# ku-fpg/ecc-ldpc

Hardware: AMD Instinct MI355X
Metric: decoded info Mbit/s @ 50 BP iters, jpl.4096.4.5, Eb/N0=2 dB (higher is better)
Workload: dtype f32; 1 GPU; jpl.4096.4.5 rate 4/5 (4096,5120) minsum flooding BP, 50 iters, Eb/N0=2.0 dB, 65536 frames/GPU/step; code_name=ldpc/hip-minsum/jpl.4096.4.5/50/4/5, batch_per_gpu=65536, parallelism=frames sharded over 1 GPU(s), tallies all-reduced

## Files before the change

ecc_ldpc_amd/csrc/fused_rows.h:

```cpp
#pragma once
#include "fused_common.h"
#ifndef LDPC_DEVICE_ONLY
#include "generated_tables.h"
#endif

namespace ldpc {

template <typename CT, int SZ>
struct DynRow {
    ctab_t p;
    __device__ __forceinline__ uint32_t lo(int k) const { return p[k] & 0xffffu; }
    __device__ __forceinline__ uint32_t hi(int k) const { return p[k] >> 16; }
};
template <typename CT, int SZ, class T, int EBEG>
struct StatRow {
    static constexpr uint32_t CPW = QcGeom<SZ>::CPW, V = QcGeom<SZ>::V, ES = sizeof(CT);
    __device__ __forceinline__ constexpr uint32_t lo(int k) const { return T::rot[EBEG + k] * CPW * ES; }
    __device__ __forceinline__ constexpr uint32_t hi(int k) const { return T::bc[EBEG + k] * V * ES; }
};
struct DynTab {
    ctab_t p;
    template <typename CT, int SZ, int EBEG> __device__ __forceinline__ DynRow<CT, SZ> row() const { return DynRow<CT, SZ>{p + EBEG}; }
    __device__ __forceinline__ DynTab rebase(uint32_t z) const { return DynTab{p + z}; }
};
template <class T>
struct StatTab {
    using Table = T;
    template <typename CT, int SZ, int EBEG> __device__ __forceinline__ StatRow<CT, SZ, T, EBEG> row() const { return {}; }
    __device__ __forceinline__ StatTab rebase(uint32_t) const { return {}; }
};
template <class Tab> struct IsStatic : std::false_type {};
template <class T> struct IsStatic<StatTab<T>> : std::true_type {};

template <class T>
struct Rounds {
    static constexpr int round_of(int e) {
        int c = 0;
        for (int j = e + 1; j < T::NEDGE; j++) c += (T::bc[j] == T::bc[e]) ? 1 : 0;
        return c;
    }
    static constexpr int num_rounds() {
        int m = 0;
        for (int e = 0; e < T::NEDGE; e++) m = round_of(e) + 1 > m ? round_of(e) + 1 : m;
        return m;
    }
    static constexpr int count(int q) {
        int c = 0;
        for (int e = 0; e < T::NEDGE; e++) c += round_of(e) == q ? 1 : 0;
        return c;
    }
    static constexpr int round0_edge(int bc) {
        for (int e = T::NEDGE - 1; e >= 0; e--)
            if (T::bc[e] == bc) return e;
        return -1;
    }
    static constexpr int nth(int q, int i) {
        int c = 0;
        for (int e = T::NEDGE - 1; e >= 0; e--)
            if (round_of(e) == q) { if (c == i) return e; c++; }
        return -1;
    }
};

template <typename CT, int SZ, class T, int Q, int I0, int I1>
__device__ __forceinline__ void round_chunk_b(char *lds, uint32_t p4, uint32_t vmask, const CT *msg, const CT *orig_rot) {
    constexpr uint32_t CPW = SZ >= 64 ? 1 : 64 / SZ, V = SZ * CPW, ES = sizeof(CT);
    asm volatile("" : "+v"(p4));
    if constexpr (Q == 0) {
        static_for<I0, I1>([&](auto ic) {
            constexpr int i = decltype(ic)::value;
            constexpr int e = Rounds<T>::nth(Q, i);
            lds_st<CT>(lds + T::bc[e] * V * ES, (p4 + T::rot[e] * CPW * ES) & vmask, msg[e] + orig_rot[T::bc[e]]);
        });
        return;
    }
    CT cur[I1 - I0];
    uint32_t adr[I1 - I0];
    static_for<I0, I1>([&](auto ic) {
        constexpr int i = decltype(ic)::value;
        constexpr int e = Rounds<T>::nth(Q, i);
        adr[i - I0] = (p4 + T::rot[e] * CPW * ES) & vmask;
        cur[i - I0] = lds_ld<CT>(lds + T::bc[e] * V * ES, adr[i - I0]);
    });
    static_for<I0, I1>([&](auto ic) {
        constexpr int i = decltype(ic)::value;
        constexpr int e = Rounds<T>::nth(Q, i);
        lds_st<CT>(lds + T::bc[e] * V * ES, adr[i - I0], msg[e] + cur[i - I0]);
    });
}
template <typename CT, int SZ, class T, int Q, int I0>
__device__ __forceinline__ void round_b(char *lds, uint32_t p4, uint32_t vmask, const CT *msg, const CT *orig_rot) {
    constexpr int CNT = Rounds<T>::count(Q), CH = 8;
    if constexpr (I0 < CNT) {
        round_chunk_b<CT, SZ, T, Q, I0, (I0 + CH < CNT ? I0 + CH : CNT)>(lds, p4, vmask, msg, orig_rot);
        round_b<CT, SZ, T, Q, I0 + CH>(lds, p4, vmask, msg, orig_rot);
    }
}

template <int RPL, int HSTEP>
__device__ __forceinline__ uint32_t row_addr(uint32_t a0, uint32_t p4, uint32_t lo, uint32_t vmask, int h) {
    if (h == 0) return a0;
    if (RPL == 2) return a0 ^ (uint32_t)HSTEP;
    return qc_wrap((p4 + HSTEP * h) + lo, vmask);
}

template <typename CT, int VARIANT, int D, int RPL, int HSTEP, bool SYNDROME_ONLY, class Row>
__device__ __forceinline__ bool rows_a(const char *lds, Row tabrow, uint32_t p4, uint32_t vmask, CT *msg) {
    asm volatile("" : "+v"(p4));
    if constexpr (SYNDROME_ONLY) LDPC_COLD_PATH();
    CT l[RPL][D];
    static_for<0, D>([&](auto kc) {
        constexpr int k = decltype(kc)::value;
        const uint32_t lo = tabrow.lo(k), hi = tabrow.hi(k);
        uint32_t a0 = qc_wrap(p4 + lo, vmask);
#pragma unroll
        for (int h = 0; h < RPL; h++) l[h][k] = lds_ld<CT>(lds + hi, row_addr<RPL, HSTEP>(a0, p4, lo, vmask, h));
    });
    bool any = false;
#pragma unroll
    for (int h = 0; h < RPL; h++) {
        bool par = false;
#pragma unroll
        for (int k = 0; k < D; k++) par ^= (l[h][k] > CT(0));
        any |= par;
    }
    if constexpr (SYNDROME_ONLY) return any;
#pragma unroll
    for (int h = 0; h < RPL; h++) {
        CT *m = msg + h * D;
        if constexpr (VARIANT == LDPC_V_MINSUM && sizeof(CT) == 4) {
            static_assert(D >= 2, "min-sum needs degree >= 2");
            uint32_t X = 0;
            float m1 = INFINITY, m2 = INFINITY;
            static_for<0, D>([&](auto kc) {
                constexpr int k = decltype(kc)::value;
                float t = l[h][k] - m[k];
                m[k] = t;
                X ^= __float_as_uint(t);
                float a = fabsf(t);
                m2 = __builtin_amdgcn_fmed3f(m1, m2, a);
                m1 = fminf(m1, a);
            });
            const uint32_t flip = (X ^ ((D & 1) ? 0x80000000u : 0u)) & 0x80000000u;
            const uint32_t c1 = __float_as_uint(0.75f * m1) ^ flip;
            const uint32_t c2 = __float_as_uint(0.75f * m2) ^ flip;
            static_for<0, D>([&](auto kc) {
                constexpr int k = decltype(kc)::value;
                float t = m[k];
                uint32_t c = (fabsf(t) == m1) ? c2 : c1;
                uint32_t tb = __float_as_uint(t);
                m[k] = __uint_as_float(__builtin_amdgcn_bitop3_b32(c, tb, 0x80000000u, 0x78));
            });
        } else {
            CT t[D];
#pragma unroll
            for (int k = 0; k < D; k++) t[k] = l[h][k] - m[k];
            cn_update<CT, VARIANT, D>(t);
#pragma unroll
            for (int k = 0; k < D; k++) m[k] = t[k];
        }
    }
    return any;
}

template <typename CT, int D, int RPL, int HSTEP, class Row>
__device__ __forceinline__ void rows_b(char *lds, Row tabrow, uint32_t p4, uint32_t vmask, const CT *msg) {
    asm volatile("" : "+v"(p4));
    CT cur[RPL][D];
    uint32_t adr[D];
    static_for<0, D>([&](auto kc) {
        constexpr int k = decltype(kc)::value;
        const uint32_t lo = tabrow.lo(k), hi = tabrow.hi(k);
        adr[k] = qc_wrap(p4 + lo, vmask);
#pragma unroll
        for (int h = 0; h < RPL; h++) cur[h][k] = lds_ld<CT>(lds + hi, row_addr<RPL, HSTEP>(adr[k], p4, lo, vmask, h));
    });
    static_for<0, D>([&](auto kc) {
        constexpr int k = decltype(kc)::value;
        const uint32_t lo = tabrow.lo(k), hi = tabrow.hi(k);
#pragma unroll
        for (int h = 0; h < RPL; h++) lds_st<CT>(lds + hi, row_addr<RPL, HSTEP>(adr[k], p4, lo, vmask, h), msg[h * D + k] + cur[h][k]);
    });
}

}
```

ecc_ldpc_amd/csrc/fused_split.hip:

```cpp
#include <stdio.h>

#ifndef SPLIT_ORIG_LDS
#define SPLIT_ORIG_LDS 12
#endif
#include "fused_split_body.h"

#ifndef SPLIT_WAVES_PER_EU
#define SPLIT_WAVES_PER_EU 4
#endif
#ifndef SPLIT_TANH_WAVES_PER_EU
#define SPLIT_TANH_WAVES_PER_EU 3
#endif

namespace ldpc {

template <typename CT, int VARIANT, class Plan, int SZ, class T>
__global__ __launch_bounds__((SplitGeom<Plan, SZ>::THREADS), (VARIANT == LDPC_V_TANH ? SPLIT_TANH_WAVES_PER_EU : SPLIT_WAVES_PER_EU))
void fused_split_kernel(FusedArgs A) {
    split_kernel_body<CT, VARIANT, Plan, SZ, T>(A);
}

bool fused_split_has(int variant, int dtype, int sz, int static_id) {
    if (dtype != LDPC_F32 || !(variant == LDPC_MINSUM || variant == LDPC_TANH)) return false;
    return (sz == 128 && static_id == 2) || (sz == 32 && static_id == 1);
}

template <int VARIANT, int SZ, class T>
static void launch_split(hipStream_t st, FusedArgs &a) {
    using G = SplitGeom<PlanAR4JA45, SZ>;
    const int grid = (a.batch + G::CPW - 1) / G::CPW;
    hipLaunchKernelGGL((fused_split_kernel<float, VARIANT, PlanAR4JA45, SZ, T>), dim3(grid), dim3(G::THREADS), 0, st, a);
}

int fused_split_launch(int variant, int sz, hipStream_t st, FusedArgs &a, KernelTimer *timer, LaunchInfo *info) {
    if (info && !a.step_mode) {
        snprintf(info->name, sizeof(info->name), "ldpc::fused_split_kernel<float, %d, ldpc::PlanAR4JA45, %d, ", variant == LDPC_MINSUM ? LDPC_V_MINSUM : LDPC_V_TANH, sz);
        info->threads = sz == 128 ? SplitGeom<PlanAR4JA45, 128>::THREADS : SplitGeom<PlanAR4JA45, 32>::THREADS;
        info->frames_per_wg = sz == 128 ? SplitGeom<PlanAR4JA45, 128>::CPW : SplitGeom<PlanAR4JA45, 32>::CPW;
    }
    if (timer && !a.step_mode) timer->begin(st);
#ifdef SPLIT_ABLATION_MINSUM128
    launch_split<LDPC_V_MINSUM, 128, TabJpl4096>(st, a);
#else
    if (sz == 128) {
        if (variant == LDPC_MINSUM) launch_split<LDPC_V_MINSUM, 128, TabJpl4096>(st, a);
        else launch_split<LDPC_V_TANH, 128, TabJpl4096>(st, a);
    } else {
        if (variant == LDPC_MINSUM) launch_split<LDPC_V_MINSUM, 32, TabJpl1024>(st, a);
        else launch_split<LDPC_V_TANH, 32, TabJpl1024>(st, a);
    }
#endif
    if (timer && !a.step_mode) timer->end(st);
    hipError_t e = hipGetLastError();
    if (e != hipSuccess) return set_error(LDPC_EHIP, "fused_split launch: %s", hipGetErrorString(e));
    return LDPC_OK;
}

}
```

ecc_ldpc_amd/csrc/fused_split_body.h:

```cpp
#pragma once
#include "fused_rows.h"

#ifndef SPLIT_ORIG_REGS
#define SPLIT_ORIG_REGS 1
#endif
#ifndef SPLIT_ORIG_LDS
#define SPLIT_ORIG_LDS 0
#endif
#ifndef SPLIT_PRIO_A
#define SPLIT_PRIO_A 2
#endif
#ifndef SPLIT_PRIO_B
#define SPLIT_PRIO_B 0
#endif
#ifndef SPLIT_CH
#define SPLIT_CH 12
#endif
#ifndef SPLIT_CH_SMALL
#define SPLIT_CH_SMALL 24
#endif

namespace ldpc {

#ifndef SPLIT_RESULT_PACKED
#define SPLIT_RESULT_PACKED 1
#endif
template <int NB, bool PACKED = (SPLIT_RESULT_PACKED && NB <= 22)> struct SplitResult;
template <int NB> struct SplitResult<NB, true> {
    struct Bits {
        uint32_t w = 0;
        __device__ __forceinline__ void set(int i, bool b) { w |= (b ? 1u : 0u) << i; }
        __device__ __forceinline__ uint32_t get(int i) const { return (w >> i) & 1u; }
    } bits;
    __device__ __forceinline__ void converge_at(int n) { bits.w = (1u << 22) | ((uint32_t)n << 23); }
    __device__ __forceinline__ bool converged() const { return (bits.w >> 22) & 1u; }
    __device__ __forceinline__ int turn() const { return (int)(bits.w >> 23); }
};
template <int NB> struct SplitResult<NB, false> {
    struct Bits {
        uint32_t w[(NB + 31) / 32] = {};
        __device__ __forceinline__ void set(int i, bool b) { w[i >> 5] |= (b ? 1u : 0u) << (i & 31); }
        __device__ __forceinline__ uint32_t get(int i) const { return (w[i >> 5] >> (i & 31)) & 1u; }
    } bits;
    uint32_t flag = 0;
    __device__ __forceinline__ void converge_at(int n) { bits = Bits{}; flag = 0x80000000u | (uint32_t)n; }
    __device__ __forceinline__ bool converged() const { return flag >> 31; }
    __device__ __forceinline__ int turn() const { return (int)(flag & 0x7fffffffu); }
};

template <class Plan, class T>
struct Split {
    static constexpr int br_of(int e) {
        int br = 0;
        for (int b = 0; b < Plan::NBR; b++) if (Plan::ebeg(b) <= e) br = b;
        return br;
    }
    static constexpr int owner_br(int br) { return Plan::owner_br(br); }
    static constexpr int owner(int e) { return owner_br(br_of(e)); }
    static constexpr int slot(int e) {
        int c = 0;
        for (int j = 0; j < e; j++) c += owner(j) == owner(e) ? 1 : 0;
        return c;
    }
    static constexpr int nmsg(int p) {
        int c = 0;
        for (int e = 0; e < T::NEDGE; e++) c += owner(e) == p ? 1 : 0;
        return c;
    }
    static constexpr int max_over_groups(int (*f)(int)) { int m = 0; for (int g = 0; g < Plan::NP; g++) m = f(g) > m ? f(g) : m; return m; }
    static constexpr int NMSG = max_over_groups(nmsg);
    static constexpr int oowner(int bc) { return owner(Rounds<T>::round0_edge(bc)); }
    static constexpr int oslot(int bc) {
        int c = 0;
        for (int j = 0; j < bc; j++) c += oowner(j) == oowner(bc) ? 1 : 0;
        return c;
    }
    static constexpr int norig(int p) {
        int c = 0;
        for (int bc = 0; bc < T::NBC; bc++) c += oowner(bc) == p ? 1 : 0;
        return c;
    }
    static constexpr int NORIG = max_over_groups(norig);
    static constexpr int count(int q, int p) {
        int c = 0;
        for (int e = 0; e < T::NEDGE; e++) c += (Rounds<T>::round_of(e) == q && owner(e) == p) ? 1 : 0;
        return c;
    }
    static constexpr int nth(int q, int p, int i) {
        int c = 0;
        for (int e = T::NEDGE - 1; e >= 0; e--)
            if (Rounds<T>::round_of(e) == q && owner(e) == p) { if (c == i) return e; c++; }
        return -1;
    }
};

template <typename CT, int VARIANT, class Plan, int SZ, class T>
struct SplitLds {
    static constexpr int V = QcGeom<SZ>::V, VT = QcGeom<SZ>::VT, THREADS = Plan::NP * VT, NW = THREADS / 64, ES = sizeof(CT);
    static constexpr int LAM_BYTES = (Plan::NBC * V * ES + 15) / 16 * 16;
    static constexpr int ORIG_OFF = LAM_BYTES + (4 * NW + 15) / 16 * 16;
    static constexpr int NOL_WANT = (VARIANT == LDPC_V_MINSUM && ES == 4 && SZ >= 64 && SPLIT_ORIG_REGS) ? SPLIT_ORIG_LDS : 0;
    static constexpr int NOL = NOL_WANT < Split<Plan, T>::NORIG ? NOL_WANT : Split<Plan, T>::NORIG;
    static constexpr int BYTES = NOL ? ORIG_OFF + NOL * THREADS * ES : LAM_BYTES + 4 * NW;
    static constexpr uint32_t orig_at(int P, int os) { return ORIG_OFF + (uint32_t)(os * THREADS + P * VT) * ES; }
};

template <typename CT, int VARIANT, int SZ, class Plan, class T, int P, int Q, int I0, int I1>
__device__ __forceinline__ void split_round_chunk(char *lds, uint32_t p4, uint32_t vmask, const CT *msg, const CT *orig_rot, const float *gllr, uint32_t r0) {
    using S = Split<Plan, T>;
    using L = SplitLds<CT, VARIANT, Plan, SZ, T>;
    constexpr uint32_t ES = sizeof(CT), CPW = QcGeom<SZ>::CPW, V = QcGeom<SZ>::V;
    asm volatile("" : "+v"(p4));
    if constexpr (Q == 0) {
        static_for<I0, I1>([&](auto ic) {
            constexpr int e = S::nth(Q, P, decltype(ic)::value);
            constexpr int ms = S::slot(e), os = S::oslot(T::bc[e]);
            CT o;
            if constexpr (SPLIT_ORIG_REGS && os < L::NOL) o = lds_ld<CT>(lds + L::orig_at(P, os), p4);
            else if constexpr (SPLIT_ORIG_REGS) o = orig_rot[os]; else o = (CT)gllr[T::bc[e] * SZ + ((r0 + T::rot[e]) % SZ)];
            lds_st<CT>(lds + T::bc[e] * V * ES, qc_wrap(p4 + T::rot[e] * CPW * ES, vmask), msg[ms] + o);
        });
        return;
    }
    CT cur[I1 - I0];
    uint32_t adr[I1 - I0];
    static_for<I0, I1>([&](auto ic) {
        constexpr int i = decltype(ic)::value;
        constexpr int e = S::nth(Q, P, i);
        adr[i - I0] = qc_wrap(p4 + T::rot[e] * CPW * ES, vmask);
        cur[i - I0] = lds_ld<CT>(lds + T::bc[e] * V * ES, adr[i - I0]);
    });
    static_for<I0, I1>([&](auto ic) {
        constexpr int i = decltype(ic)::value;
        constexpr int e = S::nth(Q, P, i);
        constexpr int ms = S::slot(e);
        lds_st<CT>(lds + T::bc[e] * V * ES, adr[i - I0], msg[ms] + cur[i - I0]);
    });
    asm volatile("" ::: "memory");
}
template <typename CT, int VARIANT, int SZ, class Plan, class T, int P, int Q, int I0>
__device__ __forceinline__ void split_round(char *lds, uint32_t p4, uint32_t vmask, const CT *msg, const CT *orig_rot, const float *gllr, uint32_t r0) {
    constexpr int CNT = Split<Plan, T>::count(Q, P), CH = SZ < 64 ? SPLIT_CH_SMALL : SPLIT_CH;
    if constexpr (I0 < CNT) {
        split_round_chunk<CT, VARIANT, SZ, Plan, T, P, Q, I0, (I0 + CH < CNT ? I0 + CH : CNT)>(lds, p4, vmask, msg, orig_rot, gllr, r0);
        split_round<CT, VARIANT, SZ, Plan, T, P, Q, I0 + CH>(lds, p4, vmask, msg, orig_rot, gllr, r0);
    }
}

template <typename CT, int VARIANT, class Plan, int SZ, class T, int P>
__device__ __forceinline__ void split_body(const FusedArgs &A, char *lds, const uint32_t tid) {
    using S = Split<Plan, T>;
    constexpr int CPW = QcGeom<SZ>::CPW, V = QcGeom<SZ>::V, VT = QcGeom<SZ>::VT;
    constexpr int N = Plan::NBC * SZ, THREADS = Plan::NP * VT, NW = THREADS / 64;
    constexpr uint32_t ES = sizeof(CT), vmask = V * ES - 1;
    constexpr int LAM_BYTES = (Plan::NBC * V * (int)ES + 15) / 16 * 16;
    if constexpr (VT != V) { if ((tid % VT) >= (uint32_t)V) return; }
    const uint32_t p4 = (tid % VT) * ES;
    struct Where {
        uint32_t sub, r0; long long frame; bool valid; size_t fN, fE;
        __device__ __forceinline__ Where(uint32_t p, int batch) {
            asm volatile("" : "+v"(p));
            const uint32_t lane = p / ES;
            sub = lane % CPW;
            r0 = lane / CPW;
            frame = (long long)blockIdx.x * CPW + sub;
            valid = frame < batch;
            fN = (size_t)(valid ? frame : 0) * N;
            fE = (size_t)(valid ? frame : 0) * Plan::NEDGE * SZ;
        }
    };
    const Where w0(p4, A.batch);
    const uint32_t r0 = w0.r0;
    const size_t fN = w0.fN, fE = w0.fE;
    CT msg[S::NMSG];
    CT orig[SPLIT_ORIG_REGS ? S::NORIG : 1];
#pragma unroll
    for (int i = 0; i < S::NMSG; i++) msg[i] = CT(0);
#pragma unroll
    for (int i = 0; i < (SPLIT_ORIG_REGS ? S::NORIG : 1); i++) orig[i] = CT(0);
    using L = SplitLds<CT, VARIANT, Plan, SZ, T>;
    static_assert(L::NOL == 0 || L::BYTES <= 65536, "LDS of one workgroup");
    auto put_orig = [&](int os, CT v) {
        if (os < L::NOL) lds_st<CT>(lds + L::orig_at(P, os), p4, v); else orig[os] = v;
    };
    typename SplitResult<(Plan::NBC + Plan::NP - 1) / Plan::NP>::Bits obits{};
    with_llr_format(A.llr_fmt, [&](auto fc) {
        constexpr int FMT = decltype(fc)::value;
        static_for<0, Plan::NBC>([&](auto bcc) {
            constexpr int bc = decltype(bcc)::value;
            if constexpr ((bc % Plan::NP) == P) {
                CT v = maybe_round_f16<CT>(load_llr_as<CT, FMT>(A.llr, fN + bc * SZ + r0), A.llr_round16);
                obits.set(bc / Plan::NP, v > CT(0));
                if (A.step_mode) v = (CT)A.st_lam[fN + bc * SZ + r0];
                lds_st<CT>(lds, p4 + (bc * V * ES), v);
            }
        });
        if (A.step_mode) {
            static_for<0, Plan::NBC>([&](auto bcc) {
                constexpr int bc = decltype(bcc)::value;
                if constexpr (SPLIT_ORIG_REGS && S::oowner(bc) == P) {
                    constexpr int e0 = Rounds<T>::round0_edge(bc);
                    constexpr int os = S::oslot(bc);
                    put_orig(os, maybe_round_f16<CT>(load_llr_as<CT, FMT>(A.llr, fN + bc * SZ + ((r0 + T::rot[e0]) % SZ)), A.llr_round16));
                }
            });
        }
    });
    if (A.step_mode) {
        static_for<0, Plan::NBR>([&](auto brc) {
            constexpr int br = decltype(brc)::value;
            if constexpr (S::owner_br(br) == P) {
                constexpr int D = Plan::deg(br);
                static_for<0, D>([&](auto kc) {
                    constexpr int k = decltype(kc)::value;
                    constexpr int ms = S::slot(Plan::ebeg(br) + k);
                    msg[ms] = (CT)A.st_ne_in[fE + (size_t)SZ * Plan::ebeg(br) + (size_t)D * r0 + k];
                });
            }
        });
    }
    __syncthreads();
    if (!A.step_mode) {
        static_for<0, Plan::NBC>([&](auto bcc) {
            constexpr int bc = decltype(bcc)::value;
            if constexpr (SPLIT_ORIG_REGS && S::oowner(bc) == P) {
                constexpr int e0 = Rounds<T>::round0_edge(bc);
                constexpr int os = S::oslot(bc);
                put_orig(os, lds_ld<CT>(lds + bc * V * ES, qc_wrap(p4 + T::rot[e0] * CPW * ES, vmask)));
            }
        });
    }

    volatile uint32_t *flags = reinterpret_cast<volatile uint32_t *>(lds + LAM_BYTES);
    constexpr uint32_t FULL = (1u << CPW) - 1;
    uint32_t done = 0;
#pragma unroll
    for (int s2 = 0; s2 < CPW; s2++) done |= ((long long)blockIdx.x * CPW + s2 < A.batch) ? 0u : (1u << s2);
    SplitResult<(Plan::NBC + Plan::NP - 1) / Plan::NP> res;
    res.bits = obits;
    const int turns = A.step_mode ? 1 : A.max_iters;

    for (int n = 0;; n++) {
        if (done == FULL) break;
        if (A.trace && !((done >> ((p4 / ES) % CPW)) & 1u)) {
            LDPC_COLD_PATH();
            const Where w(p4, A.batch);
            static_for<0, Plan::NBC>([&](auto bcc) {
                constexpr int bc = decltype(bcc)::value;
                if constexpr ((bc % Plan::NP) == P)
                    A.trace[((size_t)w.frame * (A.max_iters + 1) + n) * N + bc * SZ + w.r0] = (double)lds_ld<CT>(lds, p4 + (bc * V * ES));
            });
        }
        const bool last = (n >= turns);
        bool unsat = false;
        static_for<0, Plan::NBR>([&](auto brc) {
            constexpr int br = decltype(brc)::value;
            if constexpr (S::owner_br(br) == P) {
                constexpr int D = Plan::deg(br), ms0 = S::slot(Plan::ebeg(br));
                StatRow<CT, SZ, T, Plan::ebeg(br)> row;
                if (last) unsat |= rows_a<CT, VARIANT, D, 1, 0, true>(lds, row, p4, vmask, (CT *)nullptr);
                else unsat |= rows_a<CT, VARIANT, D, 1, 0, false>(lds, row, p4, vmask, &msg[ms0]);
            }
        });
        const unsigned long long ub = __ballot(unsat);
        uint32_t wbits = 0;
#pragma unroll
        for (int s2 = 0; s2 < CPW; s2++) {
            unsigned long long m = 0;
            for (int i = 0; i < 64; i += CPW) m |= 1ull << i;
            wbits |= ((ub & (m << s2)) != 0ull) ? (1u << s2) : 0u;
        }
        if ((tid & 63) == 0) flags[tid >> 6] = wbits;
        __syncthreads();
        uint32_t fbits = 0;
#pragma unroll
        for (int w = 0; w < NW; w++) fbits |= flags[w];
        fbits = __builtin_amdgcn_readfirstlane(fbits);
        if (A.step_mode) {
            const Where w(p4, A.batch);
            if (w.valid && w.r0 == 0 && P == 0) A.st_syn[w.frame] = ((fbits >> w.sub) & 1u) ? 0 : 1;
        } else {
            uint32_t newly = ~fbits & ~done & FULL;
            if constexpr (kVetoesNonFinite<CT, VARIANT>) {
                if (newly != 0u) {
                    LDPC_COLD_PATH();
                    bool nf = false;
                    if ((newly >> ((p4 / ES) % CPW)) & 1u)
                        static_for<0, Plan::NBC>([&](auto bcc) {
                            constexpr int bc = decltype(bcc)::value;
                            if constexpr ((bc % Plan::NP) == P) nf |= not_finite(lds_ld<CT>(lds, p4 + (bc * V * ES)));
                        });
                    __syncthreads();
                    const unsigned long long vb = __ballot(nf);
                    uint32_t vbits = 0;
#pragma unroll
                    for (int s2 = 0; s2 < CPW; s2++) {
                        unsigned long long m = 0;
                        for (int i = 0; i < 64; i += CPW) m |= 1ull << i;
                        vbits |= ((vb & (m << s2)) != 0ull) ? (1u << s2) : 0u;
                    }
                    if ((tid & 63) == 0) flags[tid >> 6] = vbits;
                    __syncthreads();
                    uint32_t veto = 0;
#pragma unroll
                    for (int w = 0; w < NW; w++) veto |= flags[w];
                    veto = __builtin_amdgcn_readfirstlane(veto) & newly;
                    __syncthreads();
                    done |= veto;
                    newly &= ~veto;
                }
            }
            if ((newly >> ((p4 / ES) % CPW)) & 1u) {
                LDPC_COLD_PATH();
                res.converge_at(n);
                static_for<0, Plan::NBC>([&](auto bcc) {
                    constexpr int bc = decltype(bcc)::value;
                    if constexpr ((bc % Plan::NP) == P) {
                        CT v = lds_ld<CT>(lds, p4 + (bc * V * ES));
                        res.bits.set(bc / Plan::NP, v > CT(0));
                    }
                });
                if (A.final_lam) {
                    const Where w(p4, A.batch);
                    static_for<0, Plan::NBC>([&](auto bcc) {
                        constexpr int bc = decltype(bcc)::value;
                        if constexpr ((bc % Plan::NP) == P) A.final_lam[w.fN + bc * SZ + w.r0] = (double)lds_ld<CT>(lds, p4 + (bc * V * ES));
                    });
                }
            }
            done |= newly;
            if (CPW > 1 && newly != 0u && done != FULL) __syncthreads();
        }
        if (last) break;
        if (done != FULL) {
            __builtin_amdgcn_s_setprio(SPLIT_PRIO_B);
            static_for<0, Rounds<T>::num_rounds()>([&](auto qc) {
                split_round<CT, VARIANT, SZ, Plan, T, P, decltype(qc)::value, 0>(lds, p4, vmask, msg, orig, reinterpret_cast<const float *>(A.llr) + fN, r0);
                __syncthreads();
            });
            __builtin_amdgcn_s_setprio(SPLIT_PRIO_A);
        }
        if (A.step_mode) break;
    }

    const Where w(p4, A.batch);
    if (!w.valid) return;
    if (A.step_mode) {
        static_for<0, Plan::NBC>([&](auto bcc) {
            constexpr int bc = decltype(bcc)::value;
            if constexpr ((bc % Plan::NP) == P) A.final_lam[w.fN + bc * SZ + w.r0] = (double)lds_ld<CT>(lds, p4 + (bc * V * ES));
        });
        static_for<0, Plan::NBR>([&](auto brc) {
            constexpr int br = decltype(brc)::value;
            if constexpr (S::owner_br(br) == P) {
                constexpr int D = Plan::deg(br);
                static_for<0, D>([&](auto kc) {
                    constexpr int k = decltype(kc)::value;
                    constexpr int ms = S::slot(Plan::ebeg(br) + k);
                    A.st_ne_out[w.fE + (size_t)SZ * Plan::ebeg(br) + (size_t)D * w.r0 + k] = (double)msg[ms];
                });
            }
        });
        return;
    }
    const bool converged = res.converged();
    if (converged) {
        static_for<0, Plan::NBC>([&](auto bcc) {
            constexpr int bc = decltype(bcc)::value;
            if constexpr ((bc % Plan::NP) == P) A.bits[w.fN + bc * SZ + w.r0] = res.bits.get(bc / Plan::NP);
        });
    } else {
        static_for<0, Plan::NBC>([&](auto bcc) {
            constexpr int bc = decltype(bcc)::value;
            if constexpr ((bc % Plan::NP) == P) A.bits[w.fN + bc * SZ + w.r0] = res.bits.get(bc / Plan::NP);
        });
        if (A.final_lam) {
            with_llr_format(A.llr_fmt, [&](auto fc) {
                constexpr int FMT = decltype(fc)::value;
                static_for<0, Plan::NBC>([&](auto bcc) {
                    constexpr int bc = decltype(bcc)::value;
                    if constexpr ((bc % Plan::NP) == P) {
                        const size_t gi = w.fN + bc * SZ + w.r0;
                        A.final_lam[gi] = (double)maybe_round_f16<CT>(load_llr_as<CT, FMT>(A.llr, gi), A.llr_round16);
                    }
                });
            });
        }
    }
    if (w.r0 == 0 && P == 0) {
        if (A.iters) A.iters[w.frame] = converged ? res.turn() : turns;
        if (A.conv) A.conv[w.frame] = converged ? 1 : 0;
    }
}

template <class Plan, int SZ> struct SplitGeom {
    static constexpr int CPW = QcGeom<SZ>::CPW, V = QcGeom<SZ>::V, VT = QcGeom<SZ>::VT, THREADS = Plan::NP * VT, NW = THREADS / 64;
    static_assert(THREADS <= 1024, "a frame's wave groups must fit one workgroup");
};

template <typename CT, int VARIANT, class Plan, int SZ, class T>
__device__ __forceinline__ void split_kernel_body(const FusedArgs &A) {
    using G = SplitGeom<Plan, SZ>;
    static_assert(SZ >= 2, "circulant size");
    __shared__ __attribute__((aligned(16))) char lds[SplitLds<CT, VARIANT, Plan, SZ, T>::BYTES];
    const uint32_t tid = threadIdx.x;
    const uint32_t pair = __builtin_amdgcn_readfirstlane(tid / G::VT);
    static_for<0, Plan::NP>([&](auto pc) {
        constexpr int P = decltype(pc)::value;
        if (pair == (uint32_t)P) split_body<CT, VARIANT, Plan, SZ, T, P>(A, lds, tid);
    });
}

}
```

Baseline: 14760 Mbit/s.

## Specialise split kernel per wave with compile-time circulant addresses and negated lambda

Instantiates the split decoder body once per 64-lane wave, so circulant rotation offsets become compile-time constants and the modulo wrap is dropped wherever a wave's rotated window cannot wrap. It also stores lambda negated, so the syndrome parity becomes an XOR of sign bits and the variable-node update folds the sign, moves the syndrome flags to an explicit LDS address space, and raises the number of orig slots kept in LDS. The aim is fewer VALU address and compare instructions per iteration, at the cost of many more template instantiations, larger code and more instruction-cache pressure.

```diff
diff --git a/ecc_ldpc_amd/csrc/fused_rows.h b/ecc_ldpc_amd/csrc/fused_rows.h
--- a/ecc_ldpc_amd/csrc/fused_rows.h
+++ b/ecc_ldpc_amd/csrc/fused_rows.h
@@ -11,12 +11,33 @@
     ctab_t p;
     __device__ __forceinline__ uint32_t lo(int k) const { return p[k] & 0xffffu; }
     __device__ __forceinline__ uint32_t hi(int k) const { return p[k] >> 16; }
+    static constexpr bool nowrap(int) { return false; }
+    static constexpr bool any_wrap(int) { return true; }
 };
 template <typename CT, int SZ, class T, int EBEG>
 struct StatRow {
     static constexpr uint32_t CPW = QcGeom<SZ>::CPW, V = QcGeom<SZ>::V, ES = sizeof(CT);
     __device__ __forceinline__ constexpr uint32_t lo(int k) const { return T::rot[EBEG + k] * CPW * ES; }
     __device__ __forceinline__ constexpr uint32_t hi(int k) const { return T::bc[EBEG + k] * V * ES; }
+    static constexpr bool nowrap(int) { return false; }
+    static constexpr bool any_wrap(int) { return true; }
+};
+template <int SZ, int WV>
+struct WaveRot {
+    static_assert(WV < 0 || (QcGeom<SZ>::CPW == 1 && SZ % 64 == 0), "wave-specialised addresses: whole waves of one frame");
+    static constexpr uint32_t rot(uint32_t r) { return WV < 0 ? r * QcGeom<SZ>::CPW : (64u * WV + r) % SZ; }
+    static constexpr bool nowrap(uint32_t r) { return WV >= 0 && rot(r) + 63 < SZ; }
+};
+template <typename CT, int SZ, class T, int EBEG, int WV>
+struct StatRowW {
+    static constexpr uint32_t V = QcGeom<SZ>::V, ES = sizeof(CT);
+    __device__ __forceinline__ constexpr uint32_t lo(int k) const { return WaveRot<SZ, WV>::rot(T::rot[EBEG + k]) * ES; }
+    __device__ __forceinline__ constexpr uint32_t hi(int k) const { return T::bc[EBEG + k] * V * ES; }
+    static constexpr bool nowrap(int k) { return WaveRot<SZ, WV>::nowrap(T::rot[EBEG + k]); }
+    static constexpr bool any_wrap(int d) {
+        for (int k = 0; k < d; k++) if (!nowrap(k)) return true;
+        return false;
+    }
 };
 struct DynTab {
     ctab_t p;
@@ -104,25 +125,40 @@
     return qc_wrap((p4 + HSTEP * h) + lo, vmask);
 }
 
-template <typename CT, int VARIANT, int D, int RPL, int HSTEP, bool SYNDROME_ONLY, class Row>
+template <typename CT, int VARIANT, int D, int RPL, int HSTEP, bool SYNDROME_ONLY, bool NEG = false, class Row>
 __device__ __forceinline__ bool rows_a(const char *lds, Row tabrow, uint32_t p4, uint32_t vmask, CT *msg) {
-    asm volatile("" : "+v"(p4));
+    const uint32_t b4 = p4;
+    if constexpr (Row::any_wrap(D)) asm volatile("" : "+v"(p4));
     if constexpr (SYNDROME_ONLY) LDPC_COLD_PATH();
     CT l[RPL][D];
     static_for<0, D>([&](auto kc) {
         constexpr int k = decltype(kc)::value;
         const uint32_t lo = tabrow.lo(k), hi = tabrow.hi(k);
-        uint32_t a0 = qc_wrap(p4 + lo, vmask);
+        uint32_t a0;
+        if constexpr (Row::nowrap(k)) a0 = b4 + lo; else a0 = qc_wrap(p4 + lo, vmask);
 #pragma unroll
         for (int h = 0; h < RPL; h++) l[h][k] = lds_ld<CT>(lds + hi, row_addr<RPL, HSTEP>(a0, p4, lo, vmask, h));
     });
     bool any = false;
-#pragma unroll
-    for (int h = 0; h < RPL; h++) {
-        bool par = false;
-#pragma unroll
-        for (int k = 0; k < D; k++) par ^= (l[h][k] > CT(0));
-        any |= par;
+    if constexpr (NEG) {
+        static_assert(VARIANT == LDPC_V_MINSUM && sizeof(CT) == 4, "negated lam: the f32 min-sum form only");
+        uint32_t odd = 0;
+#pragma unroll
+        for (int h = 0; h < RPL; h++) {
+            uint32_t px = 0;
+#pragma unroll
+            for (int k = 0; k < D; k++) px ^= __float_as_uint(l[h][k]);
+            odd |= px;
+        }
+        any = (odd >> 31) != 0u;
+    } else {
+#pragma unroll
+        for (int h = 0; h < RPL; h++) {
+            bool par = false;
+#pragma unroll
+            for (int k = 0; k < D; k++) par ^= (l[h][k] > CT(0));
+            any |= par;
+        }
     }
     if constexpr (SYNDROME_ONLY) return any;
 #pragma unroll
@@ -134,7 +170,7 @@
             float m1 = INFINITY, m2 = INFINITY;
             static_for<0, D>([&](auto kc) {
                 constexpr int k = decltype(kc)::value;
-                float t = l[h][k] - m[k];
+                float t = NEG ? (-l[h][k]) - m[k] : l[h][k] - m[k];
                 m[k] = t;
                 X ^= __float_as_uint(t);
                 float a = fabsf(t);
diff --git a/ecc_ldpc_amd/csrc/fused_split.hip b/ecc_ldpc_amd/csrc/fused_split.hip
--- a/ecc_ldpc_amd/csrc/fused_split.hip
+++ b/ecc_ldpc_amd/csrc/fused_split.hip
@@ -1,7 +1,19 @@
 #include <stdio.h>
 
 #ifndef SPLIT_ORIG_LDS
-#define SPLIT_ORIG_LDS 12
+#define SPLIT_ORIG_LDS 13
+#endif
+#ifndef SPLIT_WAVE_SPEC
+#define SPLIT_WAVE_SPEC 1
+#endif
+#ifndef SPLIT_WAVE_PHASES
+#define SPLIT_WAVE_PHASES 1
+#endif
+#ifndef SPLIT_FLAGS_LDS
+#define SPLIT_FLAGS_LDS 1
+#endif
+#ifndef SPLIT_NEG_LAM
+#define SPLIT_NEG_LAM 1
 #endif
 #include "fused_split_body.h"
 
diff --git a/ecc_ldpc_amd/csrc/fused_split_body.h b/ecc_ldpc_amd/csrc/fused_split_body.h
--- a/ecc_ldpc_amd/csrc/fused_split_body.h
+++ b/ecc_ldpc_amd/csrc/fused_split_body.h
@@ -7,6 +7,18 @@
 #ifndef SPLIT_ORIG_LDS
 #define SPLIT_ORIG_LDS 0
 #endif
+#ifndef SPLIT_WAVE_SPEC
+#define SPLIT_WAVE_SPEC 0
+#endif
+#ifndef SPLIT_WAVE_PHASES
+#define SPLIT_WAVE_PHASES 3
+#endif
+#ifndef SPLIT_FLAGS_LDS
+#define SPLIT_FLAGS_LDS 0
+#endif
+#ifndef SPLIT_NEG_LAM
+#define SPLIT_NEG_LAM 0
+#endif
 #ifndef SPLIT_PRIO_A
 #define SPLIT_PRIO_A 2
 #endif
@@ -21,6 +33,21 @@
 #endif
 
 namespace ldpc {
+
+template <typename CT, int VARIANT, int SZ>
+constexpr bool kSplitWholeWaves = VARIANT == LDPC_V_MINSUM && sizeof(CT) == 4 && QcGeom<SZ>::CPW == 1 && QcGeom<SZ>::VT == QcGeom<SZ>::V && QcGeom<SZ>::VT > 64;
+template <bool LDS_AS> struct SynFlags;
+template <> struct SynFlags<false> {
+    volatile uint32_t *p;
+    __device__ __forceinline__ explicit SynFlags(char *at) : p(reinterpret_cast<volatile uint32_t *>(at)) {}
+    __device__ __forceinline__ volatile uint32_t &operator[](uint32_t w) const { return p[w]; }
+};
+template <> struct SynFlags<true> {
+    typedef __attribute__((address_space(3))) volatile uint32_t *ptr_t;
+    ptr_t p;
+    __device__ __forceinline__ explicit SynFlags(char *at) : p((ptr_t)at) {}
+    __device__ __forceinline__ __attribute__((address_space(3))) volatile uint32_t &operator[](uint32_t w) const { return p[w]; }
+};
 
 #ifndef SPLIT_RESULT_PACKED
 #define SPLIT_RESULT_PACKED 1
@@ -105,20 +132,32 @@
     static constexpr uint32_t orig_at(int P, int os) { return ORIG_OFF + (uint32_t)(os * THREADS + P * VT) * ES; }
 };
 
-template <typename CT, int VARIANT, int SZ, class Plan, class T, int P, int Q, int I0, int I1>
-__device__ __forceinline__ void split_round_chunk(char *lds, uint32_t p4, uint32_t vmask, const CT *msg, const CT *orig_rot, const float *gllr, uint32_t r0) {
+template <typename CT, int VARIANT, int SZ, class Plan, class T, int P, int WV, int Q, int I0, int I1>
+__device__ __forceinline__ void split_round_chunk(char *lds, const uint32_t b4, uint32_t vmask, const CT *msg, const CT *orig_rot, const float *gllr, uint32_t r0) {
     using S = Split<Plan, T>;
     using L = SplitLds<CT, VARIANT, Plan, SZ, T>;
-    constexpr uint32_t ES = sizeof(CT), CPW = QcGeom<SZ>::CPW, V = QcGeom<SZ>::V;
-    asm volatile("" : "+v"(p4));
+    using R = WaveRot<SZ, WV>;
+    constexpr uint32_t ES = sizeof(CT), V = QcGeom<SZ>::V;
+    constexpr uint32_t WOFF = WV < 0 ? 0 : WV * 64 * ES;
+    constexpr bool NEG = SPLIT_NEG_LAM && kSplitWholeWaves<CT, VARIANT, SZ>;
+    constexpr bool FENCE = [] {
+        for (int i = I0; i < I1; i++) if (!R::nowrap(T::rot[S::nth(Q, P, i)])) return true;
+        return false;
+    }();
+    uint32_t p4 = b4;
+    if constexpr (FENCE) asm volatile("" : "+v"(p4));
+    auto pos = [&](auto ec) -> uint32_t {
+        constexpr uint32_t rot = T::rot[decltype(ec)::value];
+        if constexpr (R::nowrap(rot)) return b4 + R::rot(rot) * ES; else return qc_wrap(p4 + R::rot(rot) * ES, vmask);
+    };
     if constexpr (Q == 0) {
         static_for<I0, I1>([&](auto ic) {
             constexpr int e = S::nth(Q, P, decltype(ic)::value);
             constexpr int ms = S::slot(e), os = S::oslot(T::bc[e]);
             CT o;
-            if constexpr (SPLIT_ORIG_REGS && os < L::NOL) o = lds_ld<CT>(lds + L::orig_at(P, os), p4);
+            if constexpr (SPLIT_ORIG_REGS && os < L::NOL) o = lds_ld<CT>(lds + L::orig_at(P, os) + WOFF, b4);
             else if constexpr (SPLIT_ORIG_REGS) o = orig_rot[os]; else o = (CT)gllr[T::bc[e] * SZ + ((r0 + T::rot[e]) % SZ)];
-            lds_st<CT>(lds + T::bc[e] * V * ES, qc_wrap(p4 + T::rot[e] * CPW * ES, vmask), msg[ms] + o);
+            lds_st<CT>(lds + T::bc[e] * V * ES, pos(std::integral_constant<int, e>{}), NEG ? o - msg[ms] : msg[ms] + o);
         });
         return;
     }
@@ -127,27 +166,27 @@
     static_for<I0, I1>([&](auto ic) {
         constexpr int i = decltype(ic)::value;
         constexpr int e = S::nth(Q, P, i);
-        adr[i - I0] = qc_wrap(p4 + T::rot[e] * CPW * ES, vmask);
+        adr[i - I0] = pos(std::integral_constant<int, e>{});
         cur[i - I0] = lds_ld<CT>(lds + T::bc[e] * V * ES, adr[i - I0]);
     });
     static_for<I0, I1>([&](auto ic) {
         constexpr int i = decltype(ic)::value;
         constexpr int e = S::nth(Q, P, i);
         constexpr int ms = S::slot(e);
-        lds_st<CT>(lds + T::bc[e] * V * ES, adr[i - I0], msg[ms] + cur[i - I0]);
+        lds_st<CT>(lds + T::bc[e] * V * ES, adr[i - I0], NEG ? cur[i - I0] - msg[ms] : msg[ms] + cur[i - I0]);
     });
     asm volatile("" ::: "memory");
 }
-template <typename CT, int VARIANT, int SZ, class Plan, class T, int P, int Q, int I0>
+template <typename CT, int VARIANT, int SZ, class Plan, class T, int P, int WV, int Q, int I0>
 __device__ __forceinline__ void split_round(char *lds, uint32_t p4, uint32_t vmask, const CT *msg, const CT *orig_rot, const float *gllr, uint32_t r0) {
     constexpr int CNT = Split<Plan, T>::count(Q, P), CH = SZ < 64 ? SPLIT_CH_SMALL : SPLIT_CH;
     if constexpr (I0 < CNT) {
-        split_round_chunk<CT, VARIANT, SZ, Plan, T, P, Q, I0, (I0 + CH < CNT ? I0 + CH : CNT)>(lds, p4, vmask, msg, orig_rot, gllr, r0);
-        split_round<CT, VARIANT, SZ, Plan, T, P, Q, I0 + CH>(lds, p4, vmask, msg, orig_rot, gllr, r0);
+        split_round_chunk<CT, VARIANT, SZ, Plan, T, P, WV, Q, I0, (I0 + CH < CNT ? I0 + CH : CNT)>(lds, p4, vmask, msg, orig_rot, gllr, r0);
+        split_round<CT, VARIANT, SZ, Plan, T, P, WV, Q, I0 + CH>(lds, p4, vmask, msg, orig_rot, gllr, r0);
     }
 }
 
-template <typename CT, int VARIANT, class Plan, int SZ, class T, int P>
+template <typename CT, int VARIANT, class Plan, int SZ, class T, int P, int WV>
 __device__ __forceinline__ void split_body(const FusedArgs &A, char *lds, const uint32_t tid) {
     using S = Split<Plan, T>;
     constexpr int CPW = QcGeom<SZ>::CPW, V = QcGeom<SZ>::V, VT = QcGeom<SZ>::VT;
@@ -155,7 +194,11 @@
     constexpr uint32_t ES = sizeof(CT), vmask = V * ES - 1;
     constexpr int LAM_BYTES = (Plan::NBC * V * (int)ES + 15) / 16 * 16;
     if constexpr (VT != V) { if ((tid % VT) >= (uint32_t)V) return; }
-    const uint32_t p4 = (tid % VT) * ES;
+    constexpr bool NEG = SPLIT_NEG_LAM && kSplitWholeWaves<CT, VARIANT, SZ>;
+    auto stored = [](CT x) { return NEG ? CT(0) - x : x; };
+    const uint32_t b4 = (tid % (WV < 0 ? VT : 64)) * ES;
+    const uint32_t p4 = b4 + (WV < 0 ? 0 : WV * 64) * ES;
+    constexpr int WVA = (SPLIT_WAVE_PHASES & 1) ? WV : -1, WVB = (SPLIT_WAVE_PHASES & 2) ? WV : -1;
     struct Where {
         uint32_t sub, r0; long long frame; bool valid; size_t fN, fE;
         __device__ __forceinline__ Where(uint32_t p, int batch) {
@@ -192,7 +235,7 @@
                 CT v = maybe_round_f16<CT>(load_llr_as<CT, FMT>(A.llr, fN + bc * SZ + r0), A.llr_round16);
                 obits.set(bc / Plan::NP, v > CT(0));
                 if (A.step_mode) v = (CT)A.st_lam[fN + bc * SZ + r0];
-                lds_st<CT>(lds, p4 + (bc * V * ES), v);
+                lds_st<CT>(lds, p4 + (bc * V * ES), stored(v));
             }
         });
         if (A.step_mode) {
@@ -201,7 +244,7 @@
                 if constexpr (SPLIT_ORIG_REGS && S::oowner(bc) == P) {
                     constexpr int e0 = Rounds<T>::round0_edge(bc);
                     constexpr int os = S::oslot(bc);
-                    put_orig(os, maybe_round_f16<CT>(load_llr_as<CT, FMT>(A.llr, fN + bc * SZ + ((r0 + T::rot[e0]) % SZ)), A.llr_round16));
+                    put_orig(os, stored(maybe_round_f16<CT>(load_llr_as<CT, FMT>(A.llr, fN + bc * SZ + ((r0 + T::rot[e0]) % SZ)), A.llr_round16)));
                 }
             });
         }
@@ -231,7 +274,7 @@
         });
     }
 
-    volatile uint32_t *flags = reinterpret_cast<volatile uint32_t *>(lds + LAM_BYTES);
+    const SynFlags<SPLIT_FLAGS_LDS && kSplitWholeWaves<CT, VARIANT, SZ>> flags(lds + LAM_BYTES);
     constexpr uint32_t FULL = (1u << CPW) - 1;
     uint32_t done = 0;
 #pragma unroll
@@ -248,7 +291,7 @@
             static_for<0, Plan::NBC>([&](auto bcc) {
                 constexpr int bc = decltype(bcc)::value;
                 if constexpr ((bc % Plan::NP) == P)
-                    A.trace[((size_t)w.frame * (A.max_iters + 1) + n) * N + bc * SZ + w.r0] = (double)lds_ld<CT>(lds, p4 + (bc * V * ES));
+                    A.trace[((size_t)w.frame * (A.max_iters + 1) + n) * N + bc * SZ + w.r0] = (double)stored(lds_ld<CT>(lds, p4 + (bc * V * ES)));
             });
         }
         const bool last = (n >= turns);
@@ -257,9 +300,9 @@
             constexpr int br = decltype(brc)::value;
             if constexpr (S::owner_br(br) == P) {
                 constexpr int D = Plan::deg(br), ms0 = S::slot(Plan::ebeg(br));
-                StatRow<CT, SZ, T, Plan::ebeg(br)> row;
-                if (last) unsat |= rows_a<CT, VARIANT, D, 1, 0, true>(lds, row, p4, vmask, (CT *)nullptr);
-                else unsat |= rows_a<CT, VARIANT, D, 1, 0, false>(lds, row, p4, vmask, &msg[ms0]);
+                StatRowW<CT, SZ, T, Plan::ebeg(br), WVA> row;
+                if (last) unsat |= rows_a<CT, VARIANT, D, 1, 0, true, NEG>(lds, row, WVA < 0 ? p4 : b4, vmask, (CT *)nullptr);
+                else unsat |= rows_a<CT, VARIANT, D, 1, 0, false, NEG>(lds, row, WVA < 0 ? p4 : b4, vmask, &msg[ms0]);
             }
         });
         const unsigned long long ub = __ballot(unsat);
@@ -317,14 +360,14 @@
                     constexpr int bc = decltype(bcc)::value;
                     if constexpr ((bc % Plan::NP) == P) {
                         CT v = lds_ld<CT>(lds, p4 + (bc * V * ES));
-                        res.bits.set(bc / Plan::NP, v > CT(0));
+                        res.bits.set(bc / Plan::NP, NEG ? v < CT(0) : v > CT(0));
                     }
                 });
                 if (A.final_lam) {
                     const Where w(p4, A.batch);
                     static_for<0, Plan::NBC>([&](auto bcc) {
                         constexpr int bc = decltype(bcc)::value;
-                        if constexpr ((bc % Plan::NP) == P) A.final_lam[w.fN + bc * SZ + w.r0] = (double)lds_ld<CT>(lds, p4 + (bc * V * ES));
+                        if constexpr ((bc % Plan::NP) == P) A.final_lam[w.fN + bc * SZ + w.r0] = (double)stored(lds_ld<CT>(lds, p4 + (bc * V * ES)));
                     });
                 }
             }
@@ -335,7 +378,7 @@
         if (done != FULL) {
             __builtin_amdgcn_s_setprio(SPLIT_PRIO_B);
             static_for<0, Rounds<T>::num_rounds()>([&](auto qc) {
-                split_round<CT, VARIANT, SZ, Plan, T, P, decltype(qc)::value, 0>(lds, p4, vmask, msg, orig, reinterpret_cast<const float *>(A.llr) + fN, r0);
+                split_round<CT, VARIANT, SZ, Plan, T, P, WVB, decltype(qc)::value, 0>(lds, WVB < 0 ? p4 : b4, vmask, msg, orig, reinterpret_cast<const float *>(A.llr) + fN, r0);
                 __syncthreads();
             });
             __builtin_amdgcn_s_setprio(SPLIT_PRIO_A);
@@ -348,7 +391,7 @@
     if (A.step_mode) {
         static_for<0, Plan::NBC>([&](auto bcc) {
             constexpr int bc = decltype(bcc)::value;
-            if constexpr ((bc % Plan::NP) == P) A.final_lam[w.fN + bc * SZ + w.r0] = (double)lds_ld<CT>(lds, p4 + (bc * V * ES));
+            if constexpr ((bc % Plan::NP) == P) A.final_lam[w.fN + bc * SZ + w.r0] = (double)stored(lds_ld<CT>(lds, p4 + (bc * V * ES)));
         });
         static_for<0, Plan::NBR>([&](auto brc) {
             constexpr int br = decltype(brc)::value;
@@ -404,11 +447,20 @@
     static_assert(SZ >= 2, "circulant size");
     __shared__ __attribute__((aligned(16))) char lds[SplitLds<CT, VARIANT, Plan, SZ, T>::BYTES];
     const uint32_t tid = threadIdx.x;
-    const uint32_t pair = __builtin_amdgcn_readfirstlane(tid / G::VT);
-    static_for<0, Plan::NP>([&](auto pc) {
-        constexpr int P = decltype(pc)::value;
-        if (pair == (uint32_t)P) split_body<CT, VARIANT, Plan, SZ, T, P>(A, lds, tid);
-    });
+    constexpr int WPG = G::VT / 64;
+    if constexpr (SPLIT_WAVE_SPEC && kSplitWholeWaves<CT, VARIANT, SZ>) {
+        const uint32_t wave = __builtin_amdgcn_readfirstlane(tid / 64);
+        static_for<0, Plan::NP * WPG>([&](auto wc) {
+            constexpr int P = decltype(wc)::value / WPG, WV = decltype(wc)::value % WPG;
+            if (wave == (uint32_t)decltype(wc)::value) split_body<CT, VARIANT, Plan, SZ, T, P, WV>(A, lds, tid);
+        });
+    } else {
+        const uint32_t pair = __builtin_amdgcn_readfirstlane(tid / G::VT);
+        static_for<0, Plan::NP>([&](auto pc) {
+            constexpr int P = decltype(pc)::value;
+            if (pair == (uint32_t)P) split_body<CT, VARIANT, Plan, SZ, T, P, -1>(A, lds, tid);
+        });
+    }
 }
 
 }
```

Result: faster. 15910 Mbit/s, median of 6 (+7.8%).
